# jonathan-laurent/AlphaZero.jl

Measured on AMD Instinct MI355X. Metric: self-play MCTS sims/sec (Connect-Four, 4096 parallel games per GPU), higher is better.
Workload: dtype f32

## Files before the change

alphazero.jl_amd/azhip/engine.py:

```python
import ctypes as C
import os
import sys

import numpy as np

from . import _lib as L
from ._lib import EngineCfg, GameRec, MoveRec, Prof, SelfplayStats, TraceBuf, check, lib


def _vp(a):
    return a.ctypes.data_as(C.c_void_p)


def default_cfg(**kw):
    cfg = EngineCfg()
    check(lib().az_engine_cfg_init(C.byref(cfg)))
    for k, v in kw.items():
        if k == "temperature":
            xs, ys = v
            if len(xs) != len(ys) or not 1 <= len(xs) <= L.SCHED_MAX:
                raise ValueError("temperature schedule needs 1..%d breakpoints" % L.SCHED_MAX)
            cfg.temperature_len = len(xs)
            for i, (x, y) in enumerate(zip(xs, ys)):
                cfg.temperature_xs[i] = int(x)
# ... 196 lines not shown
        check(lib().az_selfplay_active(self._h, C.byref(n)))
        return n.value

    def device_bytes(self):
        n = C.c_int64()
        check(lib().az_engine_device_bytes(self._h, C.byref(n)))
        return n.value

    def release_phase(self):
        check(lib().az_engine_release_phase(self._h))

    def selfplay_end(self):
        check(lib().az_selfplay_end(self._h))

    def selfplay_aborted(self):
        n = C.c_int32()
        check(lib().az_selfplay_aborted(self._h, None, 0, C.byref(n)))
        ids = (C.c_int32 * max(n.value, 1))()
        check(lib().az_selfplay_aborted(self._h, ids, n.value, C.byref(n)))
        return [ids[i] for i in range(n.value)]

    def arena_run(self, baseline, num_games, first_game_id=0, alternate_colors=False, progress=None, traces=True):
        tb, games, moves = self._trace_buf(num_games, num_games * self.max_moves()) if traces else (None, None, None)
        rewards = np.zeros(num_games, dtype=np.float64)
        red = C.c_double()
        cb = L.PROGRESS_CB((lambda user: progress()) if progress else (lambda user: None))
        check(lib().az_arena_run(self._h, baseline._h, num_games, first_game_id, 1 if alternate_colors else 0,
                                 C.byref(tb) if traces else None, _vp(rewards), C.byref(red), cb, None))
        return games, moves, (tb.num_games if traces else 0), (tb.num_moves if traces else 0), rewards, red.value


CACHE_MAX = 4
CACHE_MAX_BYTES = int(float(os.environ.get("AZHIP_CACHE_GB", "96")) * (1 << 30))
CREATE_ENV = ("AZHIP_TOWER", "AZHIP_HEADS", "AZHIP_GRAPH", "AZHIP_XCH_EPOCH0", "AZHIP_VMM", "AZHIP_POOL_GB", "AZHIP_XCH_FAIL_AT", "AZHIP_POOLED_QUEUE",
              "AZHIP_HT_TAG_BITS", "AZHIP_HT_EPOCH0", "AZHIP_EVAL_CACHE", "AZHIP_EVAL_CACHE_LOG2", "AZHIP_VMM_KEYS", "AZHIP_TREE_ATOMIC", "AZHIP_TREE_SORT")
_cache = {}


def _cache_bytes():
    return sum(e.device_bytes() for e in _cache.values() if e._h is not None)


def _evict():
    k = next(iter(_cache))
    if os.environ.get("AZHIP_TRACE_CACHE"):
        print("azhip cache: evicting '%s' (%.1f GB)" % (k[0], _cache[k].device_bytes() / 2**30), file=sys.stderr)
    _cache.pop(k).close()


def cached_engine(role="", **kw):
    import ctypes
    cfg = default_cfg(**kw)
    key = (role, bytes(ctypes.string_at(ctypes.addressof(cfg), ctypes.sizeof(cfg))), tuple(os.environ.get(k, "") for k in CREATE_ENV))
    e = _cache.pop(key, None)
    if e is None or e._h is None:
        while len(_cache) >= CACHE_MAX:
            _evict()
        e = Engine(cfg=cfg)
        need = e.device_bytes()
        while _cache and _cache_bytes() + need > CACHE_MAX_BYTES:
            _evict()
        if os.environ.get("AZHIP_TRACE_CACHE"):
            print("azhip cache: new engine '%s' %.1f GB (cache now %.1f GB in %d engines)" % (role, need / 2**30, (_cache_bytes() + need) / 2**30, len(_cache) + 1), file=sys.stderr)
    _cache[key] = e
    return e


# ... 4 lines not shown
```

alphazero.jl_amd/csrc/azhip.hip:

```cpp
#include "engine.h"

static thread_local std::string g_err;
int fail(int code, const char* fmt, ...) {
  char buf[512];
  va_list ap;
  va_start(ap, fmt);
  vsnprintf(buf, sizeof buf, fmt, ap);
  va_end(ap);
  g_err = buf;
  return code;
}
extern "C" const char* az_last_error(void) { return g_err.c_str(); }
extern "C" int az_abi_version(void) { return AZ_ABI_VERSION; }
extern "C" int az_abi_struct_size(int32_t which) {
  switch (which) {
    case AZ_STRUCT_ENGINE_CFG: return (int)sizeof(az_engine_cfg);
    case AZ_STRUCT_MOVE_REC: return (int)sizeof(az_move_rec);
    case AZ_STRUCT_GAME_REC: return (int)sizeof(az_game_rec);
    case AZ_STRUCT_TRACE_BUF: return (int)sizeof(az_trace_buf);
    case AZ_STRUCT_SELFPLAY_STATS: return (int)sizeof(az_selfplay_stats);
    case AZ_STRUCT_SAMPLE: return (int)sizeof(az_sample);
    case AZ_STRUCT_DATASET_INFO: return (int)sizeof(az_dataset_info);
    case AZ_STRUCT_LEARNING_STATUS: return (int)sizeof(az_learning_status_t);
    case AZ_STRUCT_TRAIN_CFG: return (int)sizeof(az_train_cfg);
// ... 175 lines not shown
  if (c->num_workers < 1) return fail(AZ_ERR_BAD_ARG, "num_workers must be >= 1");
  if (c->batch_size > c->num_workers) return fail(AZ_ERR_BAD_ARG, "batch_size (%d) must be <= num_workers (%d) (src/params.jl:361-384)", c->batch_size, c->num_workers);
  if (!(c->num_iters_per_turn >= 2 || (c->num_iters_per_turn == 0 && c->oracle == AZ_ORACLE_RESNET)))
    return fail(AZ_ERR_BAD_ARG, "num_iters_per_turn must be >= 2 (with 1 the policy is 0/0, src/mcts.jl:267), or 0 with the ResNet oracle (NetworkPlayer, arena only)");
  if (!(c->flip_probability >= 0.0 && c->flip_probability <= 1.0)) return fail(AZ_ERR_BAD_ARG, "flip_probability must be in [0, 1]");
  if (c->temperature_len < 1 || c->temperature_len > AZ_SCHED_MAX) return fail(AZ_ERR_BAD_ARG, "temperature schedule needs 1..%d breakpoints", AZ_SCHED_MAX);
  if (c->reset_every < 0) return fail(AZ_ERR_BAD_ARG, "reset_every must be >= 0");
  if (c->lock_step != 0 && c->lock_step != 1) return fail(AZ_ERR_BAD_ARG, "lock_step must be 0 (free-running self-play) or 1");
  if (!(c->prior_temperature >= 0.0)) return fail(AZ_ERR_BAD_ARG, "prior_temperature must be >= 0");
  if (c->oracle == AZ_ORACLE_RESNET) {
    if (c->num_filters != 64 && c->num_filters != 128) return fail(AZ_ERR_BAD_ARG, "num_filters = %d: this build instantiates the 64- and 128-filter towers", c->num_filters);
    int hf = c->num_policy_head_filters + c->num_value_head_filters;
    if (c->num_policy_head_filters < 1 || c->num_value_head_filters < 1 || hf > c->num_filters) return fail(AZ_ERR_BAD_ARG, "head filters %d/%d unsupported (policy + value must be <= num_filters)", c->num_policy_head_filters, c->num_value_head_filters);
    if (c->num_blocks < 0 || c->num_blocks > 64) return fail(AZ_ERR_BAD_ARG, "num_blocks out of range");
    if (c->net_bf16 != 0 && c->net_bf16 != 1) return fail(AZ_ERR_BAD_ARG, "net_bf16 must be 0 or 1");
  }
  int ndev = 0;
  HIPCHK(hipGetDeviceCount(&ndev));
  if (c->device < 0 || c->device >= ndev) return fail(AZ_ERR_BAD_ARG, "device %d not available (%d visible)", c->device, ndev);
  HIPCHK(hipSetDevice(c->device));
  az_engine* e = new (std::nothrow) az_engine();
  if (!e) return fail(AZ_ERR_HIP, "out of host memory");
  e->cfg = *c; e->gi = gi; e->device = c->device; e->stream = nullptr; e->ngroups = 0; e->alloc_bytes = 0;
  e->vm_base = nullptr; e->vm_bytes = 0; e->vm_chunk = 0; e->vm_rows = 0; e->vm_chunk_nodes = 0; e->d_slot_cap = nullptr; e->vm_budget = 0; e->vm_mapped = 0;
  e->vmk_base = nullptr; e->vmk_bytes = 0; e->vmk_piece = 0; e->tree_sort = 0; e->d_perm = nullptr; e->d_perm_prev = nullptr;
  e->next_exec = 1.0;
  e->h_env = nullptr; e->h_n = nullptr; e->h_pv = nullptr; e->h_nleaf = nullptr; e->d_nleaf = nullptr; e->h_needy = nullptr; e->d_needy = nullptr;
  e->d_ec = nullptr; e->ec_mask = 0; e->ec_seq = 0; e->d_ec_claim = nullptr; e->d_Phit = nullptr; e->d_Vhit = nullptr;
  e->fr_on = false; e->fr_k = 0; e->fr_kbg = 0; e->fr_round_waves = 0; for (int i = 0; i < 4; ++i) { e->fr_s[i] = nullptr; e->fr_ev[i] = nullptr; } e->d_fr = nullptr; e->d_done = nullptr; e->d_done_off = nullptr; e->done_cap = 0;
  e->h_fr_words = nullptr; e->d_fr_words = nullptr; e->h_busy = nullptr; e->d_busy = nullptr; e->explore_k = 0; e->fr_prev_done = 0; e->fr_since_round = 0; e->fr_given_up = 0; e->fr_prev_recs = 0;
  e->h_xflag = nullptr; e->d_xflag = nullptr; e->split_off = false; e->split_registered = 0; e->xch_launches = 0;
  { const char* fa = getenv("AZHIP_XCH_FAIL_AT"); e->xch_fail_at = fa ? atoll(fa) : 0; }
  e->net_loaded = false; e->running = false; e->prof_on = false; { const char* ug = getenv("AZHIP_GRAPH"); e->use_graphs = ug ? atoi(ug) : 0; }
  e->d_phase = nullptr; e->phase_cap = 0; e->phase_n = 0; e->host_moves = true; e->last_tower[0] = 0; memset(e->tower_hist, 0, sizeof e->tower_hist); e->prof_mask = 0; e->prof_used = 0;
  memset(&e->prof, 0, sizeof e->prof);
  memset(&e->stats, 0, sizeof e->stats);
  int st = [&]() -> int {
    {
      int ncu = 0;
      HIPCHK(hipDeviceGetAttribute(&ncu, hipDeviceAttributeMultiprocessorCount, c->device));
      std::vector<uint32_t> mask((size_t)(ncu + 31) / 32, 0u);
      for (int i = 0; i < ncu; ++i) mask[(size_t)i / 32] |= 1u << (i % 32);
      if (getenv("AZHIP_POOLED_QUEUE") || ncu <= 0 || hipExtStreamCreateWithCUMask(&e->stream, (uint32_t)mask.size(), mask.data()) != hipSuccess) {
        (void)hipGetLastError();
        e->stream = nullptr;
        HIPCHK(hipStreamCreate(&e->stream));
      }
    }
    const int G = c->num_workers;
    DView& v = e->v;
    memset(&v, 0, sizeof v);
    v.G = G;
    v.max_moves = c->max_moves_per_game > 0 ? c->max_moves_per_game : gi.max_plies;
    v.max_depth = gi.max_plies + 1;
    long long cap = c->max_nodes_per_slot;
    if (cap <= 0) {
      long long plies = c->game == AZ_GAME_MANCALA ? 128 : gi.max_plies;
      cap = (long long)c->num_iters_per_turn * plies * std::max(1, c->reset_every);
      if (c->reset_every == 0) cap *= 4;
      cap = std::max<long long>(cap, 1024);
    }
    if (cap > (1LL << 30)) return fail(AZ_ERR_BAD_ARG, "max_nodes_per_slot too large");
    v.cap_nodes = (int)cap;
    int hs = 1024;
    while ((long long)hs * 2 < cap * 3) hs <<= 1;
    v.ht_size = hs;
    { const char* tb = getenv("AZHIP_HT_TAG_BITS"); const int b = tb ? atoi(tb) : 16; v.tag_mask = b >= 16 ? 0xffffu : b <= 0 ? 0u : ((1u << b) - 1u); }
// ... 89 lines not shown
    HIPCHK(hipHostGetDevicePointer((void**)&e->d_nleaf, e->h_nleaf, 0));
    HIPCHK(hipHostMalloc((void**)&e->h_needy, sizeof(int) * AZ_MAX_GROUPS, hipHostMallocMapped));
    for (int g = 0; g < AZ_MAX_GROUPS; ++g) e->h_needy[g] = 0;
    HIPCHK(hipHostGetDevicePointer((void**)&e->d_needy, e->h_needy, 0));
    AZCHK(dalloc(e, &e->d_fr, 1)); AZCHK(dalloc(e, &e->d_bg_stop, 1)); e->bg_seq = 0; e->bg_signal = false;
    HIPCHK(hipHostMalloc((void**)&e->h_busy, sizeof(int) * AZ_MAX_GROUPS, hipHostMallocMapped));
    for (int g = 0; g < AZ_MAX_GROUPS; ++g) e->h_busy[g] = -1;
    HIPCHK(hipHostGetDevicePointer((void**)&e->d_busy, e->h_busy, 0));
    { const char* ek = getenv("AZHIP_EXPLORE_K"); e->explore_k = ek ? atoi(ek) : 8; }
    HIPCHK(hipHostMalloc((void**)&e->h_fr_words, sizeof(int) * 2, hipHostMallocMapped));
    e->h_fr_words[0] = e->h_fr_words[1] = 0;
    HIPCHK(hipHostGetDevicePointer((void**)&e->d_fr_words, e->h_fr_words, 0));

    e->io_cap = std::max(G, 4096);
    AZCHK(dalloc(e, &e->d_slots, e->io_cap)); AZCHK(dalloc(e, &e->d_gids, e->io_cap)); AZCHK(dalloc(e, &e->d_roots, e->io_cap));
    AZCHK(dalloc(e, &e->d_moves, e->io_cap)); AZCHK(dalloc(e, &e->d_eta, (size_t)e->io_cap * AZ_MAX_ACTIONS));
    AZCHK(dalloc(e, &e->d_offsets, e->io_cap)); AZCHK(dalloc(e, &e->d_stage, (size_t)G * v.max_moves));
    AZCHK(dalloc(e, &e->d_keys, (size_t)2 * e->io_cap)); AZCHK(dalloc(e, &e->d_actions, e->io_cap));
    AZCHK(dalloc(e, &e->d_next, (size_t)2 * e->io_cap)); AZCHK(dalloc(e, &e->d_term, e->io_cap)); AZCHK(dalloc(e, &e->d_reward, e->io_cap));
    AZCHK(dalloc(e, &e->d_nodebuf, 512));
    AZCHK(dalloc(e, &e->d_visits, (size_t)e->io_cap * (AZ_MAX_ACTIONS + 1)));
    e->nn_cap = e->io_cap;
    AZCHK(dalloc(e, &e->d_hfeat, (size_t)e->nn_cap * gi.P * std::max(64, c->num_filters), false));
    AZCHK(dalloc(e, &e->d_X, (size_t)e->nn_cap * gi.C * gi.P)); AZCHK(dalloc(e, &e->d_A, (size_t)e->nn_cap * gi.A));
    AZCHK(dalloc(e, &e->d_P, (size_t)e->nn_cap * std::max(16, gi.APAD))); AZCHK(dalloc(e, &e->d_V, e->nn_cap)); AZCHK(dalloc(e, &e->d_Pinv, e->nn_cap));
    AZCHK(dalloc(e, &e->d_tmp_env, e->nn_cap)); AZCHK(dalloc(e, &e->d_iota, e->nn_cap)); AZCHK(dalloc(e, &e->d_ntmp, 1));
    HIPCHK(hipHostMalloc((void**)&e->h_env, sizeof(GEnv) * (size_t)e->nn_cap, hipHostMallocDefault));
    HIPCHK(hipHostMalloc((void**)&e->h_n, sizeof(int), hipHostMallocDefault));
    HIPCHK(hipHostMalloc((void**)&e->h_pv, sizeof(float) * (size_t)e->nn_cap * (gi.A + 1), hipHostMallocDefault));
    hipLaunchKernelGGL(k_iota, dim3((e->nn_cap + 255) / 256), dim3(256), 0, e->stream, e->d_iota, e->nn_cap);
    memset(&e->net, 0, sizeof e->net);
    memset(&e->net16, 0, sizeof e->net16);
    { const char* tw = getenv("AZHIP_TOWER"); e->tower_pick = tw ? atoi(tw) : 0; }
    { const char* hd = getenv("AZHIP_HEADS"); e->heads_pick = hd ? atoi(hd) : 0; }
    { const char* ep = getenv("AZHIP_XCH_EPOCH0"); e->xch_epoch = ep ? strtoull(ep, nullptr, 0) : 0; }
    { hipDeviceProp_t pr; HIPCHK(hipGetDeviceProperties(&pr, c->device)); e->num_cu = pr.multiProcessorCount; }
    AZCHK(net_set_kernel_attrs(e));
    { const char* ta = getenv("AZHIP_TREE_ATOMIC"); const int m = ta ? atoi(ta) : 0; v.bk_mode = m == 1 || m == 2 ? m : 0; }
    { const char* ts = getenv("AZHIP_TREE_SORT"); e->tree_sort = ts && atoi(ts) != 0 ? 1 : 0; }
    if (e->tree_sort) { AZCHK(dalloc(e, &e->d_perm, (size_t)2 * G)); AZCHK(dalloc(e, &e->d_perm_prev, (size_t)2 * G)); }
    int ng = c->batch_size > 0 ? G / c->batch_size : 1;
    if (ng < 1) ng = 1;
    if (ng > AZ_MAX_GROUPS) ng = AZ_MAX_GROUPS;
    while (ng > 1 && G % ng != 0) --ng;
    const int Gh = G / ng;
    const int blk_group = (Gh * gi.APAD + 255) / 256, blk_all = (G * gi.APAD + 255) / 256;
    e->stat_words = (size_t)4 * ((size_t)blk_group * ng + blk_all);
    AZCHK(dalloc(e, &v.stat, e->stat_words));
    long long* stat_base = v.stat;
    v.stat = stat_base + (size_t)4 * blk_group * ng;
    for (int g = 0; g < ng; ++g) {
      DView gv = v;
      gv.stat = stat_base + (size_t)4 * blk_group * g;
      const size_t o = (size_t)g * Gh;
      gv.G = Gh; gv.slot0 = (int)o;
      gv.sr += o; gv.game_id += o; gv.move_idx += o;
      gv.worker_sim_id += o; gv.eta += o * gi.APAD;
      gv.ht += o * hs; gv.nodes += o * v.node_stride; gv.path += o * v.max_depth;
      if (gv.slot_cap) gv.slot_cap += o;
      gv.leaf_env += o; gv.eval_slots += o; gv.bg_list += o; gv.bg_cnt += 2 * g;
      if (gv.ec) { gv.ec_claim += 2 * o; gv.Phit += o * gi.APAD; gv.Vhit += o; }
      gv.xerr = e->d_xerr + g; gv.skipped = e->d_skipped + 2 * g;
      if (e->tree_sort) {
        gv.perm = e->d_perm + o;
        hipLaunchKernelGGL(k_iota, dim3((Gh + 255) / 256), dim3(256), 0, e->stream, e->d_perm + o, Gh);
      }
// ... 478 lines not shown
  const DView& v = e->gv[g];
  hipStream_t st = e->gs[g], sn = e->gt[g];
  const bool split = st != sn;
  const int G = v.G;
  const int gb = (G * L + 255) / 256;
  const int par = (e->wave_par[g] ^= 1);
  e->stats.slot_launches += e->group_active[g];
  LAUNCH_ON(e, st, AZ_K_SELECT, G, (k_tree<Gm>), gb, 256, 0, v, e->p, (e->pending[g] || e->fr_on) ? 1 : 0, 1, par);
  e->pending[g] = true;
  hipStream_t s2 = st;
  e->bg_signal = false;
  const bool side = e->fr_on && !split && e->cfg.oracle == AZ_ORACLE_RESNET && e->fr_s[1] && st == e->fr_s[0];
  static const bool bg_stop_on = !(getenv("AZHIP_BG_STOP") && atoi(getenv("AZHIP_BG_STOP")) == 0);
  if (side) { s2 = e->fr_s[1]; HIPCHK(hipEventRecord(e->fr_ev[0], st)); ++e->bg_seq; e->bg_signal = bg_stop_on && e->fr_kbg > 0; }
  if (e->cfg.oracle == AZ_ORACLE_RESNET) {
    AZCHK(net_wave(e, g, split, e->group_active[g]));
  } else {
    LAUNCH_ON(e, st, AZ_K_SYNTH, G, (k_synth_oracle<Gm>), (G + 255) / 256, 256, 0, v, e->p, sim_idx, par);
  }
  if (e->fr_on) {
    FRArgs fa;
    fa.st = e->d_fr; fa.done = e->d_done; fa.done_off = e->d_done_off;
    fa.recs = e->d_phase ? e->d_phase : e->d_stage; fa.recs_cap = e->d_phase ? (long long)e->phase_cap : (long long)e->v.G * e->v.max_moves;
    fa.done_cap = e->done_cap; fa.total_games = e->total_games; fa.first_game_id = (uint32_t)e->first_game_id; fa.group = g; fa.host_words = e->d_fr_words;
    static const int bg_prio = getenv("AZHIP_BG_PRIO") ? atoi(getenv("AZHIP_BG_PRIO")) : 0;
    hipStream_t s3 = side ? e->fr_s[2] : s2;
    if (side) { HIPCHK(hipStreamWaitEvent(s2, e->fr_ev[0], 0)); HIPCHK(hipStreamWaitEvent(s3, e->fr_ev[0], 0)); }
    { DView mv = v; mv.low_prio = bg_prio ? 0 : 1; LAUNCH_ON(e, s3, AZ_K_MOVE, G, (k_move_fr<Gm>), (G + 255) / 256, 256, 0, mv, e->p, fa); }
    if (e->fr_kbg > 0) {
      AZCHK(ec_next_launch(e, &e->gv[g]));
      DView bv = e->gv[g];
      bv.run_k = e->fr_kbg; bv.low_prio = bg_prio ? 0 : 1;
      if (side && e->bg_signal) { bv.bg_stop = e->d_bg_stop; bv.bg_seq = e->bg_seq; }
      LAUNCH_ON(e, s2, AZ_K_EXPAND, G, (k_tree<Gm>), gb, 256, 0, bv, e->p, 0, 1, par ^ 1);
    }
    if (side) {
      HIPCHK(hipEventRecord(e->fr_ev[1], s2)); HIPCHK(hipStreamWaitEvent(st, e->fr_ev[1], 0));
      HIPCHK(hipEventRecord(e->fr_ev[2], s3)); HIPCHK(hipStreamWaitEvent(st, e->fr_ev[2], 0));
    }
    else if (split && e->cfg.oracle == AZ_ORACLE_RESNET) HIPCHK(hipStreamWaitEvent(st, e->ev_net[g], 0));
  }
  return AZ_OK;
}
template <class Gm> static int recover_split(az_engine* e) {
  AZCHK(sync_all(e));
  *e->h_xflag = 0;
  int xerr[AZ_MAX_GROUPS + 1], skipped[2 * (AZ_MAX_GROUPS + 1)];
  HIPCHK(hipMemcpy(xerr, e->d_xerr, sizeof xerr, hipMemcpyDeviceToHost));
  HIPCHK(hipMemcpy(skipped, e->d_skipped, sizeof skipped, hipMemcpyDeviceToHost));
  HIPCHK(hipMemsetAsync(e->d_xerr, 0, sizeof xerr, e->stream));
  HIPCHK(hipMemsetAsync(e->d_skipped, 0, sizeof skipped, e->stream));
  HIPCHK(hipStreamSynchronize(e->stream));
  bool any = false;
  for (int g = 0; g < e->ngroups; ++g) any = any || xerr[g] == DERR_EXCHANGE;
  if (!any) return AZ_OK;
  e->split_off = true;
  e->stats.tower_fallbacks++;
  for (int g = 0; g < e->ngroups; ++g) {
    e->wave_par[g] ^= (skipped[2 * g] & 1);
    if (skipped[2 * g + 1]) e->pending[g] = true;
  }
  if (e->cfg.oracle == AZ_ORACLE_RESNET)
    for (int g = 0; g < e->ngroups; ++g)
      if (e->pending[g] && e->group_active[g] > 0) {
        AZCHK(net_wave(e, g, e->gs[g] != e->gt[g], e->group_active[g]));
        if (e->fr_on && e->gs[g] != e->gt[g]) HIPCHK(hipStreamWaitEvent(e->gs[g], e->ev_net[g], 0));
      }
// ... 887 lines not shown
```

alphazero.jl_amd/csrc/engine.h:

```cpp
#pragma once
#include <hip/hip_runtime.h>

#include <algorithm>
#include <chrono>
#include <cmath>
#include <cstdarg>
#include <cstdio>
#include <cstring>
#include <new>
#include <string>
#include <map>
#include <mutex>
#include <vector>
#include <unordered_set>

#include "../../include/az_numerics.h"
#include "../../include/azhip.h"
#include "games.h"
#include "resnet.h"
#include "resnet16.h"
#include "resnet16b.h"
#include "tree.h"

int fail(int code, const char* fmt, ...);
// ... 43 lines not shown
  hipEvent_t ev_tree[AZ_MAX_GROUPS], ev_net[AZ_MAX_GROUPS];
  float* g_hfeat[AZ_MAX_GROUPS];
  unsigned long long* xch[AZ_MAX_GROUPS + 1]; unsigned long long xch_epoch;
  int* d_xerr; int* d_skipped;
  int* h_needy; int* d_needy;
  int* h_nleaf; int* d_nleaf;
  int* h_xflag; int* d_xflag;
  bool split_off;
  long long xch_fail_at, xch_launches;
  int split_registered;
  std::vector<void*> allocs;
  size_t alloc_bytes;
  char* vm_base; size_t vm_bytes, vm_chunk; int vm_rows, vm_chunk_nodes;
  std::vector<hipMemGenericAllocationHandle_t> vm_handles; std::vector<char*> vm_at;
  std::vector<int> h_slot_cap, h_node_count; int* d_slot_cap; int* d_node_count; size_t vm_budget, vm_mapped;
  char* vmk_base; size_t vmk_bytes, vmk_piece; std::vector<uint8_t> vmk_granule;
  int tree_sort; int* d_perm; long long* d_perm_prev;
  ECEnt* d_ec; uint32_t ec_mask; uint32_t ec_seq; int* d_ec_claim; float* d_Phit; float* d_Vhit;
  size_t stat_words; std::vector<long long> h_stat;
  std::vector<int32_t> aborted_ids;
  std::vector<void*> net_allocs;
  bool net_loaded;
  std::vector<float> blob;
  NetDev net;
  Net16bDev net16b;
  Net16Dev net16;
  uint16_t* d_geo[7];
  int nts;
  int ntm;
  long long tower_hist[4];
  char last_tower[96];
  int heads_pick;
  int tower_pick;
  int num_cu;
  int nn_cap;
  float* d_hfeat; float* d_X; float* d_A; float* d_P; float* d_V; float* d_Pinv;
  GEnv* d_tmp_env; int* d_iota; int* d_ntmp;
  GEnv* h_env; int* h_n; float* h_pv;
  int* d_slots; uint32_t* d_gids; GEnv* d_roots; uint32_t* d_moves; double* d_eta; int* d_offsets;
  az_move_rec* d_stage; unsigned long long* d_keys; int* d_actions; unsigned long long* d_next; signed char* d_term; float* d_reward;
  char* d_nodebuf;
  int* d_visits;
  int io_cap;
  bool running;
  int total_games, next_game, first_game_id, games_done, wave_in_move, active_slots;
  std::map<int, hipGraphExec_t> wave_graphs; int use_graphs;
  bool pending[AZ_MAX_GROUPS];
  int wave_par[AZ_MAX_GROUPS];
  int group_active[AZ_MAX_GROUPS];
  bool fr_on;
  int fr_k, fr_kbg, fr_round_waves;
  hipStream_t fr_s[4]; hipEvent_t fr_ev[4];
  FRState* d_fr; az_game_rec* d_done; long long* d_done_off; int done_cap;
  int* h_busy; int* d_busy;
  int explore_k;
  int* d_bg_stop; int bg_seq; bool bg_signal;
  int* h_fr_words; int* d_fr_words;
  int fr_prev_done, fr_since_round, fr_given_up; long long fr_prev_recs;
  std::vector<az_game_rec> h_done; std::vector<long long> h_done_off;
  std::vector<az_game_rec> q_games;
  std::vector<az_move_rec> q_moves;
  az_move_rec* d_phase; int64_t phase_cap, phase_n; bool host_moves;
  std::vector<az_game_rec> ph_games;
  std::vector<int64_t> ph_off;
  az_selfplay_stats stats;
  std::chrono::steady_clock::time_point t_begin;
// ... 115 lines not shown
```

alphazero.jl_amd/csrc/net_impl.h:

```cpp
#pragma once
#include "engine.h"

template <class Gm, int F, bool PLANES_ONLY = false> static int set_kernel_attrs_f() {
  HIPCHK(hipFuncSetAttribute(reinterpret_cast<const void*>(&k_tower16<Gm, F, false>), hipFuncAttributeMaxDynamicSharedMemorySize, T16<Gm, F>::BYTES));
  HIPCHK(hipFuncSetAttribute(reinterpret_cast<const void*>(&k_tower16<Gm, F, true>), hipFuncAttributeMaxDynamicSharedMemorySize, T16<Gm, F>::BYTES));
  if constexpr (NTM<Gm> > 0) {
    HIPCHK(hipFuncSetAttribute(reinterpret_cast<const void*>(&k_tower16<Gm, F, false, NTM<Gm>>), hipFuncAttributeMaxDynamicSharedMemorySize, T16<Gm, F, NTM<Gm>>::BYTES));
    HIPCHK(hipFuncSetAttribute(reinterpret_cast<const void*>(&k_tower16<Gm, F, true, NTM<Gm>>), hipFuncAttributeMaxDynamicSharedMemorySize, T16<Gm, F, NTM<Gm>>::BYTES));
  }
  if constexpr (F == 64) {
    HIPCHK(hipFuncSetAttribute(reinterpret_cast<const void*>(&k_tower16x2<Gm, F, false>), hipFuncAttributeMaxDynamicSharedMemorySize, T16P<Gm, F>::BYTES));
    HIPCHK(hipFuncSetAttribute(reinterpret_cast<const void*>(&k_tower16x2<Gm, F, true>), hipFuncAttributeMaxDynamicSharedMemorySize, T16P<Gm, F>::BYTES));
    HIPCHK(hipFuncSetAttribute(reinterpret_cast<const void*>(&k_tower16x2<Gm, F, false, 10, 9>), hipFuncAttributeMaxDynamicSharedMemorySize, T16P<Gm, F, 10, 9>::BYTES));
    HIPCHK(hipFuncSetAttribute(reinterpret_cast<const void*>(&k_tower16x2<Gm, F, true, 10, 9>), hipFuncAttributeMaxDynamicSharedMemorySize, T16P<Gm, F, 10, 9>::BYTES));
    HIPCHK(hipFuncSetAttribute(reinterpret_cast<const void*>(&k_tower16x2m<Gm, F, false>), hipFuncAttributeMaxDynamicSharedMemorySize, T16P<Gm, F>::BYTES));
    HIPCHK(hipFuncSetAttribute(reinterpret_cast<const void*>(&k_tower16x2c<Gm, F, false>), hipFuncAttributeMaxDynamicSharedMemorySize, T16P<Gm, F>::BYTES));
    HIPCHK(hipFuncSetAttribute(reinterpret_cast<const void*>(&k_tower16x2c<Gm, F, true>), hipFuncAttributeMaxDynamicSharedMemorySize, T16P<Gm, F>::BYTES));
  }
  HIPCHK(hipFuncSetAttribute(reinterpret_cast<const void*>(&k_tower16b<Gm, F, false, 11>), hipFuncAttributeMaxDynamicSharedMemorySize, T16B<Gm, F, 11>::BYTES));
  HIPCHK(hipFuncSetAttribute(reinterpret_cast<const void*>(&k_tower16b<Gm, F, true, 11>), hipFuncAttributeMaxDynamicSharedMemorySize, T16B<Gm, F, 11>::BYTES));
  HIPCHK(hipFuncSetAttribute(reinterpret_cast<const void*>(&k_tower16b<Gm, F, false, NTS<Gm>>), hipFuncAttributeMaxDynamicSharedMemorySize, T16B<Gm, F, NTS<Gm>>::BYTES));
  HIPCHK(hipFuncSetAttribute(reinterpret_cast<const void*>(&k_tower16b<Gm, F, true, NTS<Gm>>), hipFuncAttributeMaxDynamicSharedMemorySize, T16B<Gm, F, NTS<Gm>>::BYTES));
  if constexpr (F == 128) {
    HIPCHK(hipFuncSetAttribute(reinterpret_cast<const void*>(&k_tower16b<Gm, F, false, 22>), hipFuncAttributeMaxDynamicSharedMemorySize, T16B<Gm, F, 22>::BYTES));
// ... 193 lines not shown
      LAUNCH_ON(e, st, AZ_K_TOWER, n_max, (k_tower16<Gm, F, FROM_PLANES, NTM<Gm>>), (n_max + TM::TB - 1) / TM::TB, THR16, (TM::BYTES), e->net16, envs, eslots, n_ptr, n_max, X, hfeat);
    }
  } else if (tw == 3)
    LAUNCH_ON(e, st, AZ_K_TOWER, n_max, (k_tower16<Gm, F, FROM_PLANES, NTS<Gm>>), (n_max + TB3 - 1) / TB3, THR16, LDS3, e->net16, envs, eslots, n_ptr, n_max, X, hfeat);
  else if (tw == 16)
    LAUNCH_ON(e, st, AZ_K_TOWER, n_max, (k_tower16<Gm, F, FROM_PLANES>), (n_max + TB16 - 1) / TB16, THR16, LDS16, e->net16, envs, eslots, n_ptr, n_max, X, hfeat);
  else
    LAUNCH_ON(e, st, AZ_K_TOWER, n_max, (k_tower<Gm, F, FROM_PLANES>), gt, TowerCfg<F>::THREADS, TowerLds<F>::BYTES, e->net, envs, eslots, n_ptr, n_max, X, hfeat);
  return launch_heads<Gm, F>(e, st, hfeat, envs, eslots, n_ptr, n_max, Amask, Pout, Vout, Pinv, pstride);
}
template <class Gm, bool FROM_PLANES>
static int launch_net(az_engine* e, hipStream_t st, float* hfeat, const GEnv* envs, const int* eslots, const int* n_ptr, int n_max, const float* X,
                      const float* Amask, float* Pout, float* Vout, float* Pinv, int pstride) {
  if (e->cfg.num_filters == 128) return launch_net_f<Gm, 128, FROM_PLANES>(e, st, hfeat, envs, eslots, n_ptr, n_max, X, Amask, Pout, Vout, Pinv, pstride);
  return launch_net_f<Gm, 64, FROM_PLANES>(e, st, hfeat, envs, eslots, n_ptr, n_max, X, Amask, Pout, Vout, Pinv, pstride);
}


template <class Gm, int F> static int wave_net_f(az_engine* e, int g, bool split, int nmax) {
  constexpr int L = Gm::APAD, TB = TOWER_ROWS / Gm::P;
  const DView& v = e->gv[g];
  hipStream_t st = e->gs[g], sn = e->gt[g];
  const int G = v.G;
  if (split) { HIPCHK(hipEventRecord(e->ev_tree[g], st)); HIPCHK(hipStreamWaitEvent(sn, e->ev_tree[g], 0)); }
  constexpr int TB16 = T16<Gm, F>::TB, THR16 = T16<Gm, F>::THREADS, LDS16 = T16<Gm, F>::BYTES;
  constexpr int TB3 = T16<Gm, F, NTS<Gm>>::TB, LDS3 = T16<Gm, F, NTS<Gm>>::BYTES;
  constexpr int TB21 = T16P<Gm, 64>::TB, THR21 = T16P<Gm, 64>::THREADS, LDS21 = T16P<Gm, 64>::BYTES;
  const int N = std::max(1, std::min(G, nmax));
  const int* nev = v.n_eval + e->wave_par[g];
  const int* const eslots = v.eval_slots + (size_t)e->wave_par[g] * v.eval_stride;
  int npick = N;
  if (v.nleaf_host) { const int seen = ((volatile int*)e->h_nleaf)[g]; if (seen >= 0) npick = std::max(1, std::min(N, seen + seen / 8 + 8)); }
  int tw = pick_tower<Gm, F>(e, npick, N);
  if (tw == 21 && e->fr_on && e->ngroups == 1 && e->tower_pick == 0 && e->fr_kbg > 0 && v.nleaf_host && v.needy_host) {
    const int cu = e->num_cu > 0 ? e->num_cu : 256;
    const int seen = ((volatile int*)e->h_nleaf)[g], needy = ((volatile int*)e->h_needy)[g];
    if (seen > 0) {
      const int wgs = (seen + TB21 - 1) / TB21, rounds = (wgs + cu - 1) / cu, bg = (std::max(needy, 0) * L + 255) / 256;
      if (wgs > rounds * (cu - bg) - 14) tw = 20;
    }
  }
  note_tower(e, tw, F);
  e->next_exec = tower_exec_frac<Gm, F>(e, tw);
  if (e->cfg.net_bf16) {
    constexpr int TBb = T16B<Gm, F>::TB, THRb = T16B<Gm, F>::THREADS, LDSb = T16B<Gm, F>::BYTES, TBb3 = T16B<Gm, F, NTS<Gm>>::TB, LDSb3 = T16B<Gm, F, NTS<Gm>>::BYTES;
    if (tw == 22) {
      constexpr int TB22 = T16B<Gm, F, 22>::TB, LDS22 = T16B<Gm, F, 22>::BYTES;
      if constexpr (F == 128) LAUNCH_ON(e, sn, AZ_K_TOWER, N, (k_tower16b<Gm, F, false, 22>), (N + TB22 - 1) / TB22, THRb, LDS22, e->net16b, v.leaf_env, eslots, nev, N, (const float*)nullptr, e->g_hfeat[g]);
    } else if (tw == 3) LAUNCH_ON(e, sn, AZ_K_TOWER, N, (k_tower16b<Gm, F, false, NTS<Gm>>), (N + TBb3 - 1) / TBb3, THRb, LDSb3, e->net16b, v.leaf_env, eslots, nev, N, (const float*)nullptr, e->g_hfeat[g]);
    else LAUNCH_ON(e, sn, AZ_K_TOWER, N, (k_tower16b<Gm, F, false, 11>), (N + TBb - 1) / TBb, THRb, LDSb, e->net16b, v.leaf_env, eslots, nev, N, (const float*)nullptr, e->g_hfeat[g]);
  } else if (tw == 2) {
    if constexpr (F == 128) {
      unsigned long long* xa; unsigned long long ep;
      AZCHK(xch_slot<Gm>(e, e->g_hfeat[g], &xa, &ep));
      LAUNCH_ON(e, sn, AZ_K_TOWER, N, (k_tower16s<Gm, F, false>), 2 * ((N + TB3 - 1) / TB3), (T16S<Gm, F>::THREADS), LDS3, e->net16, v.leaf_env, eslots, nev, N, (const float*)nullptr, e->g_hfeat[g],
                xa, ep, v.xerr, e->d_xflag);
    }
  } else if (tw == 20) {
    if constexpr (F == 64)
      LAUNCH_ON(e, sn, AZ_K_TOWER, N, (k_tower16x2c<Gm, F, false>), (N + TB21 - 1) / TB21, THR21, LDS21, e->net16, v.leaf_env, eslots, nev, N, (const float*)nullptr, e->g_hfeat[g], 0);
  } else if (tw == 21 || tw == 19) {
    if constexpr (F == 64) {
      static const bool mixed_on = getenv("AZHIP_TOWER_MIXED") && atoi(getenv("AZHIP_TOWER_MIXED")) != 0;
      using T19 = T16P<Gm, 64, 10, 9>;
      static const bool rounds_on = getenv("AZHIP_TOWER_ROUNDS") && atoi(getenv("AZHIP_TOWER_ROUNDS")) != 0;
      const int cu = e->num_cu > 0 ? e->num_cu : 256, first = cu * TB21;
      const int seen = v.nleaf_host ? ((volatile int*)e->h_nleaf)[g] : -1;
      if (tw == 19) {
        LAUNCH_ON(e, sn, AZ_K_TOWER, N, (k_tower16x2<Gm, F, false, 10, 9>), (N + T19::TB - 1) / T19::TB, (T19::THREADS), (T19::BYTES), e->net16, v.leaf_env, eslots, nev, N, (const float*)nullptr, e->g_hfeat[g], 0);
      } else if (mixed_on && !rounds_on && e->tower_pick == 0 && N > first && seen > first && seen + 16 <= first + cu * T19::TB) {
        e->next_exec = (first * tower_exec_frac<Gm, F>(e, 21) + (seen - first) * tower_exec_frac<Gm, F>(e, 19)) / (double)seen;
        LAUNCH_ON(e, sn, AZ_K_TOWER, N, (k_tower16x2m<Gm, F, false>), cu + (N - first + T19::TB - 1) / T19::TB, THR21, LDS21, e->net16, v.leaf_env, eslots, nev, N, (const float*)nullptr, e->g_hfeat[g], cu);
        snprintf(e->last_tower, sizeof e->last_tower, "k_tower16x2m<%s,%d>", Gm::ID == 0 ? "ConnectFour" : Gm::ID == 1 ? "TicTacToe" : "Mancala", F);
      } else if (rounds_on && e->tower_pick == 0 && N > first && seen > first && seen + 16 <= first + cu * T19::TB) {
        LAUNCH_ON(e, sn, AZ_K_TOWER, first, (k_tower16x2<Gm, F, false>), cu, THR21, LDS21, e->net16, v.leaf_env, eslots, nev, N, (const float*)nullptr, e->g_hfeat[g], 0);
        e->next_exec = tower_exec_frac<Gm, F>(e, 19);
        LAUNCH_ON(e, sn, AZ_K_TOWER, N - first, (k_tower16x2<Gm, F, false, 10, 9>), (N - first + T19::TB - 1) / T19::TB, (T19::THREADS), (T19::BYTES), e->net16, v.leaf_env, eslots, nev, N, (const float*)nullptr, e->g_hfeat[g], first);
      } else {
        LAUNCH_ON(e, sn, AZ_K_TOWER, N, (k_tower16x2<Gm, F, false>), (N + TB21 - 1) / TB21, THR21, LDS21, e->net16, v.leaf_env, eslots, nev, N, (const float*)nullptr, e->g_hfeat[g], 0);
      }
    }
  } else if (tw == 7) {
    if constexpr (NTM<Gm> > 0) {
      using TM = T16<Gm, F, NTM<Gm>>;
      LAUNCH_ON(e, sn, AZ_K_TOWER, N, (k_tower16<Gm, F, false, NTM<Gm>>), (N + TM::TB - 1) / TM::TB, THR16, (TM::BYTES), e->net16, v.leaf_env, eslots, nev, N, (const float*)nullptr, e->g_hfeat[g]);
    }
  } else if (tw == 3)
    LAUNCH_ON(e, sn, AZ_K_TOWER, N, (k_tower16<Gm, F, false, NTS<Gm>>), (N + TB3 - 1) / TB3, THR16, LDS3, e->net16, v.leaf_env, eslots, nev, N, (const float*)nullptr, e->g_hfeat[g]);
  else if (tw == 16)
    LAUNCH_ON(e, sn, AZ_K_TOWER, N, (k_tower16<Gm, F, false>), (N + TB16 - 1) / TB16, THR16, LDS16, e->net16, v.leaf_env, eslots, nev, N, (const float*)nullptr, e->g_hfeat[g]);
  else
    LAUNCH_ON(e, sn, AZ_K_TOWER, N, (k_tower<Gm, F, false>), (N + TB - 1) / TB, TowerCfg<F>::THREADS, TowerLds<F>::BYTES, e->net, v.leaf_env, eslots, nev, N, (const float*)nullptr, e->g_hfeat[g]);
  const bool fr = e->fr_on && split;
  if (e->bg_signal) {
    HIPCHK(hipEventRecord(e->fr_ev[3], sn));
    HIPCHK(hipStreamWaitEvent(e->fr_s[3], e->fr_ev[3], 0));
    hipLaunchKernelGGL(k_set_word, dim3(1), dim3(1), 0, e->fr_s[3], e->d_bg_stop, e->bg_seq);
  }
  if (split && !fr) { HIPCHK(hipEventRecord(e->ev_net[g], sn)); HIPCHK(hipStreamWaitEvent(st, e->ev_net[g], 0)); }
  AZCHK((launch_heads<Gm, F>(e, fr ? sn : st, e->g_hfeat[g], v.leaf_env, eslots, nev, N, (const float*)nullptr, v.Pout, v.Vout, (float*)nullptr, L)));
  if (fr) HIPCHK(hipEventRecord(e->ev_net[g], sn));
  return AZ_OK;
}
template <class Gm> static int wave_net(az_engine* e, int g, bool split, int nmax) {
  return e->cfg.num_filters == 128 ? wave_net_f<Gm, 128>(e, g, split, nmax) : wave_net_f<Gm, 64>(e, g, split, nmax);
}

#define AZ_NET_GAME_TU(Gm, sfx)                                                                                              \
  int net_set_kernel_attrs_##sfx(az_engine* e) { return set_kernel_attrs<Gm>(e); }                                                      \
  int net_launch_##sfx(az_engine* e, hipStream_t st, bool from_planes, float* hfeat, const GEnv* envs, const int* eslots,    \
// ... 13 lines not shown
```

alphazero.jl_amd/csrc/tree.h:

```cpp
#pragma once
#include <hip/hip_runtime.h>
#include <stdint.h>
#include <type_traits>
#include "../../include/az_numerics.h"
#include "../../include/azhip.h"
#include "games.h"

enum { LEAF_NONE = 0, LEAF_NEW = 1, LEAF_TERMINAL = 2 };
enum { DERR_NODE_POOL = 1, DERR_HASH_FULL = 2, DERR_DEPTH = 3, DERR_MOVES = 4, DERR_NO_ROOT = 5 };

struct DParams {
  double gamma, cpuct, eps, alpha, prior_temp;
  int nsims, temp_len;
  int temp_xs[AZ_SCHED_MAX];
  double temp_ys[AZ_SCHED_MAX];
  uint64_t seed;
  int oracle, reset_every;
  double flip_p;
  int retire;
};

enum { SR_ACTIVE = 1, SR_MS_SHIFT = 8 };
struct alignas(64) SlotRec {
  unsigned long long root_a, root_b;
// ... 204 lines not shown
      return (int)__shfl((int)idx1, base + fm) - 1;
    }
    if (fd != 99) { *ins = (h0 + (uint32_t)(i * L + fd)) & H1; return -1; }
  }
  dev_fail(v, DERR_HASH_FULL);
  *ins = 0;
  return -1;
}

template <class Gm>
__device__ inline void arm_noise(const DView& v, const DParams& p, int slot, const GEnv& env) {
  constexpr int L = Gm::APAD;
  uint32_t m = Gm::mask(env);
  int n = __popc(m);
  double eta[AZ_MAX_ACTIONS];
  az_rng r = az_rng_make(p.seed, v.game_id[slot], v.move_idx[slot], AZ_RNG_NOISE);
  az_dirichlet(&r, n, p.alpha, eta);
  int k = 0;
  for (int a = 0; a < L; ++a) {
    double e = 0.0;
    if (a < Gm::A && ((m >> a) & 1)) e = eta[k++];
    v.eta[(size_t)slot * L + a] = e;
  }
}

template <class Gm> __device__ inline void set_link(char* nd, int act, uint32_t link) {
  using NL = NodeL<Gm>;
  ((uint16_t*)(nd + NL::OFF_LO))[act] = (uint16_t)(link & 0xffff);
  typename NL::hi_t* hp = (typename NL::hi_t*)(nd + NL::OFF_HI);
  *hp = (typename NL::hi_t)((*hp & ~((typename NL::hi_t)3 << (2 * act))) | ((typename NL::hi_t)(link >> 16) << (2 * act)));
}

struct KArgs { DView v; DParams p; };
template <class Gm>
__global__ void __launch_bounds__(256) __attribute__((amdgpu_num_vgpr(160))) k_tree(DView v_arg, DParams p_arg, int do_backup, int do_select, int par) {
  if (!v_arg.low_prio) __builtin_amdgcn_s_setprio(3);
  const DView& v = v_arg;
  constexpr int L = Gm::APAD;
  using NL = NodeL<Gm>;
  __shared__ int s_new[4], s_hit[4], s_evl[4], s_sims[4], s_trav[4], s_need[4], s_base, s_nbase;
  const int tid = blockIdx.x * blockDim.x + threadIdx.x;
  const int lgrp = tid / L, lane = tid % L;
  const int wl = threadIdx.x & 63, w = threadIdx.x >> 6, gbase = wl & ~(L - 1);
  int nlive = v.G;
  const int* map = v.perm;
  if (v.fr && !do_backup && v.bg_list) { nlive = v.bg_cnt[par ^ 1]; map = v.bg_list + (size_t)(par ^ 1) * v.eval_stride; }
  const bool live = lgrp < nlive;
  const int slot_in = live ? (map ? map[lgrp] : lgrp) : 0;
  const bool links_ok = v.cap_nodes <= LINK_MAX;
  unsigned long long* dbg = (v.dbg && blockIdx.x == 0 && threadIdx.x == 0) ? v.dbg : nullptr;
  if (dbg) dbg[0] = __builtin_readcyclecounter();
  if (__hip_atomic_load(v.xerr, __ATOMIC_RELAXED, __HIP_MEMORY_SCOPE_AGENT) == (int)DERR_EXCHANGE) {
    if (blockIdx.x == 0 && threadIdx.x == 0 && (do_backup || !v.fr)) atomicAdd(v.skipped + (do_select ? 0 : 1), 1);
    return;
  }

  const SlotRec s0 = v.sr[slot_in];
  unsigned long long st = (v.path + (size_t)slot_in * v.max_depth)[lane < v.max_depth ? lane : 0];
  GEnv lenv = v.leaf_env[slot_in];
  int kind = s0.leaf_kd & 3, depth = (s0.leaf_kd >> 2) & 0x0fffffff, e0 = s0.eidx, nc = s0.node_count;
  GEnv root0 = s0.root();
  uint32_t epoch0 = s0.epoch, ins = s0.leaf_ins;
  int ridx = s0.root_idx, active0 = s0.active;
  int claim0 = -1; uint32_t cmeta0 = 0;
  if (v.ec) { const int2 c2 = ((const int2*)v.ec_claim)[slot_in]; claim0 = c2.x; cmeta0 = (uint32_t)c2.y; }
#define AZ_PIN(x) asm volatile("" : "+v"(x))
  AZ_PIN(kind); AZ_PIN(depth); AZ_PIN(e0); AZ_PIN(nc); AZ_PIN(st); AZ_PIN(root0.a); AZ_PIN(root0.b); AZ_PIN(root0.fin);
  AZ_PIN(epoch0); AZ_PIN(ins); AZ_PIN(claim0); AZ_PIN(cmeta0); AZ_PIN(lenv.a); AZ_PIN(lenv.b); AZ_PIN(lenv.fin); AZ_PIN(ridx); AZ_PIN(active0);
  const bool mine = live && !(v.fr && kind != LEAF_NONE && (!do_backup || ((s0.leaf_kd >> 30) & 1) == par));
  if (!(do_backup && mine)) kind = LEAF_NONE;
  const int nc_in = nc, ridx_in = ridx;
  const bool inrec = lane < Gm::A;
  float Pans = 0.f, Vans = 0.f;
  if (kind == LEAF_NEW) {
    Pans = e0 >= 0 ? v.Pout[(size_t)e0 * L + lane] : v.Phit[(size_t)slot_in * L + lane];
    Vans = e0 >= 0 ? v.Vout[e0] : v.Vhit[slot_in];
  }
  const bool searching = mine && (active0 & SR_ACTIVE);
  int msims = active0 >> SR_MS_SHIFT;
  int done_sims = 0, done_trav = 0;
  int n_sel = 0, n_trav = 0, n_evl = 0, n_hit = 0;
  bool retired = false, ishit = false;
  int claim = -1; uint32_t cmeta = 0;

  for (int it = 0;; ++it) {
    KArgs ka;
    {
      auto kp = __builtin_amdgcn_kernarg_segment_ptr();
      asm volatile("" : "+s"(kp));
      __builtin_memcpy(&ka, (const void*)kp, sizeof(KArgs));
    }
    const DView& v = ka.v;
    const DParams& p = ka.p;
    int slot = slot_in; asm volatile("" : "+v"(slot));
    unsigned long long* const path = v.path + (size_t)slot * v.max_depth;
    if (kind != LEAF_NONE) {
      double q = 0.0;
      bool ok = true;
      if (kind == LEAF_NEW) {
        const int idx = nc;
        if (it == 0 && v.ec && claim0 >= 0) {
// ... 233 lines not shown
    if (ts) {
      long long* sp = v.stat + (size_t)blockIdx.x * 4;
      sp[0] += ts; sp[1] += tt; sp[2] += te; sp[3] += toth;
    }
    if (blockIdx.x == 0 && (do_backup || !v.fr)) {
      if (v.nleaf_host && do_select) __hip_atomic_store(v.nleaf_host, v.n_eval[par ^ 1], __ATOMIC_RELAXED, __HIP_MEMORY_SCOPE_SYSTEM);
      v.n_eval[par ^ 1] = 0;
      if (v.bg_cnt) {
        if (v.busy_host && v.run_k && !v.fr && do_backup) __hip_atomic_store(v.busy_host, v.bg_cnt[par ^ 1], __ATOMIC_RELAXED, __HIP_MEMORY_SCOPE_SYSTEM);
        if (v.needy_host && v.fr && do_backup) __hip_atomic_store(v.needy_host, v.bg_cnt[par ^ 1], __ATOMIC_RELAXED, __HIP_MEMORY_SCOPE_SYSTEM);
        v.bg_cnt[par ^ 1] = 0;
      }
    }
  }
  __syncthreads();
  if (dbg) dbg[5] = __builtin_readcyclecounter();
  if (isnew) {
    int base = s_base;
    for (int i = 0; i < w; ++i) base += s_new[i];
    const int e = base + __popcll(bal & ((1ULL << wl) - 1ULL));
    sr->eidx = e;
    (v.eval_slots + (size_t)par * v.eval_stride)[e] = slot;
  }
  if (needy && v.fr) {
    int base = s_nbase;
    for (int i = 0; i < w; ++i) base += s_need[i];
    (v.bg_list + (size_t)par * v.eval_stride)[base + __popcll(baln & ((1ULL << wl) - 1ULL))] = slot;
  }
  if (v.ec && head && kind == LEAF_NEW) ((int2*)v.ec_claim)[slot] = make_int2(ishit ? -1 : claim, ishit ? 0 : (int)cmeta);
  if (dbg) dbg[6] = __builtin_readcyclecounter();
}

template <class Gm>
__host__ __device__ inline float rollout_value(GEnv g, uint64_t seed, uint32_t game_id, uint32_t move, uint32_t sim) {
  const bool wp = Gm::white_playing(g);
  az_rng r = az_rng_make(seed, game_id, move, AZ_RNG_ROLLOUT);
  r.ctr[3] = sim * 1024u;
  double wr = 0.0;
  for (int ply = 0; ply < 1024 && !(g.fin & 1); ++ply) {
    const uint32_t m = Gm::mask(g);
    int acts[AZ_MAX_ACTIONS], n = 0;
    for (int a = 0; a < Gm::A; ++a) if ((m >> a) & 1) acts[n++] = a;
    int k = (int)(az_rng_f64(&r) * (double)n);
    if (k >= n) k = n - 1;
    Gm::play(g, acts[k]);
    wr = (double)Gm::white_reward(g);
  }
  return (float)(wp ? wr : -wr);
}

template <class Gm>
__global__ void __launch_bounds__(256) k_synth_oracle(DView v, DParams p, uint32_t sim_idx, int par) {
  __builtin_amdgcn_s_setprio(3);
  constexpr int L = Gm::APAD;
  const int e = blockIdx.x * blockDim.x + threadIdx.x;
  if (e >= v.n_eval[par]) return;
  const int* const eslots = v.eval_slots + (size_t)par * v.eval_stride;
  const GEnv env = v.leaf_env[eslots[e]];
  const uint32_t m = Gm::mask(env);
  float P[L];
  float V = 0.f;
  if (p.oracle == AZ_ORACLE_UNIFORM || p.oracle == AZ_ORACLE_ROLLOUT) {
    const float u = (float)(1.0 / (double)__popc(m));
    for (int a = 0; a < L; ++a) P[a] = ((m >> a) & 1) ? u : 0.f;
    if (p.oracle == AZ_ORACLE_ROLLOUT) {
      const int slot = eslots[e];
// ... 363 lines not shown
```

Before: 8.892 million.

## Add low-VGPR background tree kernel to share CUs with tower instead of downgrading

```diff
diff --git a/alphazero.jl_amd/azhip/engine.py b/alphazero.jl_amd/azhip/engine.py
--- a/alphazero.jl_amd/azhip/engine.py
+++ b/alphazero.jl_amd/azhip/engine.py
@@ -252,7 +252,7 @@
 
 CACHE_MAX = 4
 CACHE_MAX_BYTES = int(float(os.environ.get("AZHIP_CACHE_GB", "96")) * (1 << 30))
-CREATE_ENV = ("AZHIP_TOWER", "AZHIP_HEADS", "AZHIP_GRAPH", "AZHIP_XCH_EPOCH0", "AZHIP_VMM", "AZHIP_POOL_GB", "AZHIP_XCH_FAIL_AT", "AZHIP_POOLED_QUEUE",
+CREATE_ENV = ("AZHIP_TOWER", "AZHIP_TOWER_MIXED", "AZHIP_HEADS", "AZHIP_GRAPH", "AZHIP_XCH_EPOCH0", "AZHIP_VMM", "AZHIP_POOL_GB", "AZHIP_XCH_FAIL_AT", "AZHIP_POOLED_QUEUE",
               "AZHIP_HT_TAG_BITS", "AZHIP_HT_EPOCH0", "AZHIP_EVAL_CACHE", "AZHIP_EVAL_CACHE_LOG2", "AZHIP_VMM_KEYS", "AZHIP_TREE_ATOMIC", "AZHIP_TREE_SORT")
 _cache = {}
 
diff --git a/alphazero.jl_amd/csrc/azhip.hip b/alphazero.jl_amd/csrc/azhip.hip
--- a/alphazero.jl_amd/csrc/azhip.hip
+++ b/alphazero.jl_amd/csrc/azhip.hip
@@ -231,7 +231,7 @@
   e->h_xflag = nullptr; e->d_xflag = nullptr; e->split_off = false; e->split_registered = 0; e->xch_launches = 0;
   { const char* fa = getenv("AZHIP_XCH_FAIL_AT"); e->xch_fail_at = fa ? atoll(fa) : 0; }
   e->net_loaded = false; e->running = false; e->prof_on = false; { const char* ug = getenv("AZHIP_GRAPH"); e->use_graphs = ug ? atoi(ug) : 0; }
-  e->d_phase = nullptr; e->phase_cap = 0; e->phase_n = 0; e->host_moves = true; e->last_tower[0] = 0; memset(e->tower_hist, 0, sizeof e->tower_hist); e->prof_mask = 0; e->prof_used = 0;
+  e->d_phase = nullptr; e->phase_cap = 0; e->phase_n = 0; e->host_moves = true; e->last_tower[0] = 0; e->bg_share = false; e->tower_mixed = 0; memset(e->tower_hist, 0, sizeof e->tower_hist); e->prof_mask = 0; e->prof_used = 0;
   memset(&e->prof, 0, sizeof e->prof);
   memset(&e->stats, 0, sizeof e->stats);
   int st = [&]() -> int {
@@ -387,6 +387,7 @@
     memset(&e->net, 0, sizeof e->net);
     memset(&e->net16, 0, sizeof e->net16);
     { const char* tw = getenv("AZHIP_TOWER"); e->tower_pick = tw ? atoi(tw) : 0; }
+    { const char* mx = getenv("AZHIP_TOWER_MIXED"); e->tower_mixed = mx ? (atoi(mx) != 0) : 0; }
     { const char* hd = getenv("AZHIP_HEADS"); e->heads_pick = hd ? atoi(hd) : 0; }
     { const char* ep = getenv("AZHIP_XCH_EPOCH0"); e->xch_epoch = ep ? strtoull(ep, nullptr, 0) : 0; }
     { hipDeviceProp_t pr; HIPCHK(hipGetDeviceProperties(&pr, c->device)); e->num_cu = pr.multiProcessorCount; }
@@ -931,7 +932,8 @@
       DView bv = e->gv[g];
       bv.run_k = e->fr_kbg; bv.low_prio = bg_prio ? 0 : 1;
       if (side && e->bg_signal) { bv.bg_stop = e->d_bg_stop; bv.bg_seq = e->bg_seq; }
-      LAUNCH_ON(e, s2, AZ_K_EXPAND, G, (k_tree<Gm>), gb, 256, 0, bv, e->p, 0, 1, par ^ 1);
+      if (e->bg_share && e->cfg.oracle == AZ_ORACLE_RESNET) LAUNCH_ON(e, s2, AZ_K_EXPAND, G, (k_tree_bg<Gm>), gb, 256, 0, bv, e->p, par ^ 1);
+      else LAUNCH_ON(e, s2, AZ_K_EXPAND, G, (k_tree<Gm>), gb, 256, 0, bv, e->p, 0, 1, par ^ 1);
     }
     if (side) {
       HIPCHK(hipEventRecord(e->fr_ev[1], s2)); HIPCHK(hipStreamWaitEvent(st, e->fr_ev[1], 0));
diff --git a/alphazero.jl_amd/csrc/engine.h b/alphazero.jl_amd/csrc/engine.h
--- a/alphazero.jl_amd/csrc/engine.h
+++ b/alphazero.jl_amd/csrc/engine.h
@@ -99,6 +99,8 @@
   char last_tower[96];
   int heads_pick;
   int tower_pick;
+  int tower_mixed;
+  bool bg_share;
   int num_cu;
   int nn_cap;
   float* d_hfeat; float* d_X; float* d_A; float* d_P; float* d_V; float* d_Pinv;
diff --git a/alphazero.jl_amd/csrc/net_impl.h b/alphazero.jl_amd/csrc/net_impl.h
--- a/alphazero.jl_amd/csrc/net_impl.h
+++ b/alphazero.jl_amd/csrc/net_impl.h
@@ -249,12 +249,13 @@
   int npick = N;
   if (v.nleaf_host) { const int seen = ((volatile int*)e->h_nleaf)[g]; if (seen >= 0) npick = std::max(1, std::min(N, seen + seen / 8 + 8)); }
   int tw = pick_tower<Gm, F>(e, npick, N);
-  if (tw == 21 && e->fr_on && e->ngroups == 1 && e->tower_pick == 0 && e->fr_kbg > 0 && v.nleaf_host && v.needy_host) {
+  e->bg_share = e->tower_mixed != 0;
+  if (tw == 21 && e->fr_on && e->ngroups == 1 && e->fr_kbg > 0 && v.nleaf_host && v.needy_host) {
     const int cu = e->num_cu > 0 ? e->num_cu : 256;
     const int seen = ((volatile int*)e->h_nleaf)[g], needy = ((volatile int*)e->h_needy)[g];
     if (seen > 0) {
       const int wgs = (seen + TB21 - 1) / TB21, rounds = (wgs + cu - 1) / cu, bg = (std::max(needy, 0) * L + 255) / 256;
-      if (wgs > rounds * (cu - bg) - 14) tw = 20;
+      if (wgs > rounds * (cu - bg) - 14) e->bg_share = true;
     }
   }
   note_tower(e, tw, F);
@@ -278,21 +279,15 @@
       LAUNCH_ON(e, sn, AZ_K_TOWER, N, (k_tower16x2c<Gm, F, false>), (N + TB21 - 1) / TB21, THR21, LDS21, e->net16, v.leaf_env, eslots, nev, N, (const float*)nullptr, e->g_hfeat[g], 0);
   } else if (tw == 21 || tw == 19) {
     if constexpr (F == 64) {
-      static const bool mixed_on = getenv("AZHIP_TOWER_MIXED") && atoi(getenv("AZHIP_TOWER_MIXED")) != 0;
       using T19 = T16P<Gm, 64, 10, 9>;
-      static const bool rounds_on = getenv("AZHIP_TOWER_ROUNDS") && atoi(getenv("AZHIP_TOWER_ROUNDS")) != 0;
       const int cu = e->num_cu > 0 ? e->num_cu : 256, first = cu * TB21;
       const int seen = v.nleaf_host ? ((volatile int*)e->h_nleaf)[g] : -1;
       if (tw == 19) {
         LAUNCH_ON(e, sn, AZ_K_TOWER, N, (k_tower16x2<Gm, F, false, 10, 9>), (N + T19::TB - 1) / T19::TB, (T19::THREADS), (T19::BYTES), e->net16, v.leaf_env, eslots, nev, N, (const float*)nullptr, e->g_hfeat[g], 0);
-      } else if (mixed_on && !rounds_on && e->tower_pick == 0 && N > first && seen > first && seen + 16 <= first + cu * T19::TB) {
+      } else if (e->tower_mixed && e->fr_on && e->ngroups == 1 && e->tower_pick == 0 && N > first && seen > first && seen + 16 <= first + cu * T19::TB) {
         e->next_exec = (first * tower_exec_frac<Gm, F>(e, 21) + (seen - first) * tower_exec_frac<Gm, F>(e, 19)) / (double)seen;
         LAUNCH_ON(e, sn, AZ_K_TOWER, N, (k_tower16x2m<Gm, F, false>), cu + (N - first + T19::TB - 1) / T19::TB, THR21, LDS21, e->net16, v.leaf_env, eslots, nev, N, (const float*)nullptr, e->g_hfeat[g], cu);
         snprintf(e->last_tower, sizeof e->last_tower, "k_tower16x2m<%s,%d>", Gm::ID == 0 ? "ConnectFour" : Gm::ID == 1 ? "TicTacToe" : "Mancala", F);
-      } else if (rounds_on && e->tower_pick == 0 && N > first && seen > first && seen + 16 <= first + cu * T19::TB) {
-        LAUNCH_ON(e, sn, AZ_K_TOWER, first, (k_tower16x2<Gm, F, false>), cu, THR21, LDS21, e->net16, v.leaf_env, eslots, nev, N, (const float*)nullptr, e->g_hfeat[g], 0);
-        e->next_exec = tower_exec_frac<Gm, F>(e, 19);
-        LAUNCH_ON(e, sn, AZ_K_TOWER, N - first, (k_tower16x2<Gm, F, false, 10, 9>), (N - first + T19::TB - 1) / T19::TB, (T19::THREADS), (T19::BYTES), e->net16, v.leaf_env, eslots, nev, N, (const float*)nullptr, e->g_hfeat[g], first);
       } else {
         LAUNCH_ON(e, sn, AZ_K_TOWER, N, (k_tower16x2<Gm, F, false>), (N + TB21 - 1) / TB21, THR21, LDS21, e->net16, v.leaf_env, eslots, nev, N, (const float*)nullptr, e->g_hfeat[g], 0);
       }
diff --git a/alphazero.jl_amd/csrc/tree.h b/alphazero.jl_amd/csrc/tree.h
--- a/alphazero.jl_amd/csrc/tree.h
+++ b/alphazero.jl_amd/csrc/tree.h
@@ -260,8 +260,9 @@
 }
 
 struct KArgs { DView v; DParams p; };
-template <class Gm>
-__global__ void __launch_bounds__(256) __attribute__((amdgpu_num_vgpr(160))) k_tree(DView v_arg, DParams p_arg, int do_backup, int do_select, int par) {
+template <class Gm, bool BG>
+__device__ __forceinline__ void tree_launch(const DView& v_arg, const DParams& p_arg, const int do_backup_arg, const int do_select_arg, const int par) {
+  const int do_backup = BG ? 0 : do_backup_arg, do_select = BG ? 1 : do_select_arg;
   if (!v_arg.low_prio) __builtin_amdgcn_s_setprio(3);
   const DView& v = v_arg;
   constexpr int L = Gm::APAD;
@@ -284,17 +285,17 @@
   }
 
   const SlotRec s0 = v.sr[slot_in];
-  unsigned long long st = (v.path + (size_t)slot_in * v.max_depth)[lane < v.max_depth ? lane : 0];
-  GEnv lenv = v.leaf_env[slot_in];
+  unsigned long long st = BG ? 0ULL : (v.path + (size_t)slot_in * v.max_depth)[lane < v.max_depth ? lane : 0];
+  GEnv lenv = BG ? GEnv{0, 0, 0} : v.leaf_env[slot_in];
   int kind = s0.leaf_kd & 3, depth = (s0.leaf_kd >> 2) & 0x0fffffff, e0 = s0.eidx, nc = s0.node_count;
   GEnv root0 = s0.root();
   uint32_t epoch0 = s0.epoch, ins = s0.leaf_ins;
   int ridx = s0.root_idx, active0 = s0.active;
   int claim0 = -1; uint32_t cmeta0 = 0;
-  if (v.ec) { const int2 c2 = ((const int2*)v.ec_claim)[slot_in]; claim0 = c2.x; cmeta0 = (uint32_t)c2.y; }
+  if (!BG && v.ec) { const int2 c2 = ((const int2*)v.ec_claim)[slot_in]; claim0 = c2.x; cmeta0 = (uint32_t)c2.y; }
 #define AZ_PIN(x) asm volatile("" : "+v"(x))
-  AZ_PIN(kind); AZ_PIN(depth); AZ_PIN(e0); AZ_PIN(nc); AZ_PIN(st); AZ_PIN(root0.a); AZ_PIN(root0.b); AZ_PIN(root0.fin);
-  AZ_PIN(epoch0); AZ_PIN(ins); AZ_PIN(claim0); AZ_PIN(cmeta0); AZ_PIN(lenv.a); AZ_PIN(lenv.b); AZ_PIN(lenv.fin); AZ_PIN(ridx); AZ_PIN(active0);
+  AZ_PIN(kind); AZ_PIN(nc); AZ_PIN(root0.a); AZ_PIN(root0.b); AZ_PIN(root0.fin); AZ_PIN(epoch0); AZ_PIN(ridx); AZ_PIN(active0);
+  if (!BG) { AZ_PIN(depth); AZ_PIN(e0); AZ_PIN(st); AZ_PIN(ins); AZ_PIN(claim0); AZ_PIN(cmeta0); AZ_PIN(lenv.a); AZ_PIN(lenv.b); AZ_PIN(lenv.fin); }
   const bool mine = live && !(v.fr && kind != LEAF_NONE && (!do_backup || ((s0.leaf_kd >> 30) & 1) == par));
   if (!(do_backup && mine)) kind = LEAF_NONE;
   const int nc_in = nc, ridx_in = ridx;
@@ -594,6 +595,15 @@
 }
 
 template <class Gm>
+__global__ void __launch_bounds__(256) __attribute__((amdgpu_num_vgpr(160))) k_tree(DView v_arg, DParams p_arg, int do_backup, int do_select, int par) {
+  tree_launch<Gm, false>(v_arg, p_arg, do_backup, do_select, par);
+}
+template <class Gm>
+__global__ void __launch_bounds__(256) __attribute__((amdgpu_num_vgpr(56))) k_tree_bg(DView v_arg, DParams p_arg, int par) {
+  tree_launch<Gm, true>(v_arg, p_arg, 0, 1, par);
+}
+
+template <class Gm>
 __host__ __device__ inline float rollout_value(GEnv g, uint64_t seed, uint32_t game_id, uint32_t move, uint32_t sim) {
   const bool wp = Gm::white_playing(g);
   az_rng r = az_rng_make(seed, game_id, move, AZ_RNG_ROLLOUT);
```

New measurement: 8.880 million. Within noise of the previous version (-0.1%).
